# google-deepmind/dqn_zoo

Hardware: NVIDIA H100
Metric: learner_grad_steps_per_sec (higher is better)
Workload: dtype f32 (f64 sum tree)

## Files before the change

### dqn_zoo_b200/_lib.py

```python

import ctypes as C
import os

from dqn_zoo_b200 import _build

i32, i64, f32, f64, u64 = C.c_int32, C.c_int64, C.c_float, C.c_double, C.c_uint64
vp = C.c_void_p

DZ_FLAG_BAD_VALUE, DZ_FLAG_BAD_INDEX, DZ_FLAG_BAD_TARGET, DZ_FLAG_ROOT_ZERO, DZ_FLAG_NONFINITE_WEIGHT = 1, 2, 4, 8, 16
DZ_FLAG_FRAME_POOL_FULL = 32
AGENT_KINDS = {'dqn': 0, 'double_q': 1, 'prioritized': 2, 'c51': 3, 'qrdqn': 4, 'rainbow': 5, 'iqn': 6}
OPTIMIZERS = {'adam': 0, 'rmsprop': 1}


class ReplayView(C.Structure):
  _fields_ = [('d_obs', vp), ('d_action', vp), ('d_reward', vp), ('d_discount', vp), ('capacity', i64),
              ('obs_bytes', i64), ('obs_stride', i64), ('d_tree', vp), ('first_leaf', i64), ('d_live', vp),
              ('d_id_at', vp), ('d_ids', vp), ('d_flags', vp),
              ('d_frames', vp), ('frame_bytes', i64), ('frame_stride', i64), ('obs_channels', i64),
              ('frame_capacity', i64), ('d_planes', vp), ('d_refcount', vp), ('d_hashes', vp), ('d_table', vp),
              ('table_size', i64), ('d_free', vp), ('d_pool_counters', vp), ('d_add_staging', vp)]


class AddRecord(C.Structure):
# ... 86 lines not shown
    'dz_learner_sync_target': (i32, [vp, vp]),
    'dz_test_u8_to_unit': (i32, [vp, vp]),
    'dz_atari_preprocess': (i32, [vp, vp, i32, vp, vp, vp, vp, i32, vp, i32, vp]),
    'dz_atari_preprocess_band_rows': (i32, []),
    'dz_jax_uniform': (i32, [vp, vp, i32, vp, vp]),
    'dz_test_threefry2x32': (i32, [C.c_uint32, C.c_uint32, C.c_uint32, C.c_uint32, vp]),
    'dz_test_learner_buffer': (i32, [vp, C.c_char_p, vp, vp]),
    'dz_test_copy': (i32, [vp, vp, i64, vp]),
    'dz_test_learner_trace': (i32, [vp, C.c_char_p, vp]),
    'dz_test_learner_mma_path': (i32, [vp, C.c_char_p, C.POINTER(i32)]),
    'dz_debug_timeline': (i32, [vp]),
    'dz_test_tc_pgemm_work': (i64, [i32, i32, i32]),
    'dz_test_tc_pgemm': (i32, [vp, i32, i32, i32, vp, i32, i32, i32, i32, i32, vp, vp, i64, i64, i32, i64, vp, i32, vp]),
    'dz_test_umma_gemm': (i32, [vp, i32, vp, i32, i32, i32, i32, i32, vp, i32, i32, vp, i32, vp, vp, vp, vp]),
    'dz_test_umma_gemm_path': (i32, [vp, i32, vp, i32, i32, i32, i32, i32, vp, i32, i32, vp, i32, vp, vp, vp, i32, vp]),
}

EXPORTS = tuple(_SIGNATURES)


def library_path():
  return _build.LIB_PATH


def _load():
  path = library_path()
  if not os.path.exists(path):
    raise ImportError('dqn_zoo_b200: %s is missing — run `python -c "import __graft_entry__ as g; g.build()"` '
                      '(there is no CPU fallback)' % path)
  lib = C.CDLL(path)
# ... 17 lines not shown
```

### dqn_zoo_b200/csrc/dz_tc.cuh

```cuda
#pragma once
#include <cuda_runtime.h>
#include <stdint.h>

namespace dz {
namespace tc {

__device__ __forceinline__ void mma_16x8x8(float (&d)[4], const uint32_t (&a)[4], const uint32_t (&b)[2]) {
  asm volatile("mma.sync.aligned.m16n8k8.row.col.f32.tf32.tf32.f32 {%0, %1, %2, %3}, {%4, %5, %6, %7}, {%8, %9}, {%0, %1, %2, %3};"
               : "+f"(d[0]), "+f"(d[1]), "+f"(d[2]), "+f"(d[3])
               : "r"(a[0]), "r"(a[1]), "r"(a[2]), "r"(a[3]), "r"(b[0]), "r"(b[1]));
}

template <int MT, int NT, class AOff, class BOff>
__device__ __forceinline__ void warp_kstep_3xtf32(float (&sum)[MT][NT][4], const uint8_t* a_hi, const uint8_t* a_lo,
                                                  const uint8_t* b_hi, const uint8_t* b_lo, int m0, int n0, int k0,
                                                  AOff a_off, BOff b_off) {
  const int lane = threadIdx.x & 31, g = lane >> 2, t = lane & 3;
  uint32_t ah[MT][4], al[MT][4];
#pragma unroll
  for (int mt = 0; mt < MT; ++mt) {
#pragma unroll
    for (int q = 0; q < 4; ++q) {
      const uint32_t o = a_off(m0 + mt * 16 + g + (q & 1) * 8, k0 + t + (q >> 1) * 4);
      ah[mt][q] = *reinterpret_cast<const uint32_t*>(a_hi + o);
      al[mt][q] = a_lo ? *reinterpret_cast<const uint32_t*>(a_lo + o) : 0u;
    }
  }
#pragma unroll
  for (int nt = 0; nt < NT; ++nt) {
    uint32_t bh[2], bl[2];
#pragma unroll
    for (int q = 0; q < 2; ++q) {
      const uint32_t o = b_off(n0 + nt * 8 + g, k0 + t + q * 4);
      bh[q] = *reinterpret_cast<const uint32_t*>(b_hi + o);
      bl[q] = *reinterpret_cast<const uint32_t*>(b_lo + o);
    }
#pragma unroll
    for (int mt = 0; mt < MT; ++mt) {
      float p[4] = {0.f, 0.f, 0.f, 0.f};
      if (a_lo) mma_16x8x8(p, al[mt], bh);
      mma_16x8x8(p, ah[mt], bl);
      mma_16x8x8(p, ah[mt], bh);
#pragma unroll
      for (int e = 0; e < 4; ++e) sum[mt][nt][e] += p[e];
    }
  }
}

__device__ __forceinline__ uint64_t wgmma_desc_sw128(uint32_t smem_addr) {
  return (uint64_t)((smem_addr & 0x3FFFFu) >> 4) | ((uint64_t)1 << 16) | ((uint64_t)(1024 >> 4) << 32) | ((uint64_t)1 << 62);
}
__device__ __forceinline__ void wgmma_fence() { asm volatile("wgmma.fence.sync.aligned;" ::: "memory"); }
__device__ __forceinline__ void wgmma_commit() { asm volatile("wgmma.commit_group.sync.aligned;" ::: "memory"); }
template <int N>
__device__ __forceinline__ void wgmma_wait() { asm volatile("wgmma.wait_group.sync.aligned %0;" ::"n"(N) : "memory"); }
template <int NA>
__device__ __forceinline__ void wgmma_fence_acc(float (&d)[NA]) {
#pragma unroll
  for (int e = 0; e < NA; ++e) asm volatile("" : "+f"(d[e])::"memory");
}

// ... 82 lines not shown
```

### dqn_zoo_b200/csrc/dz_umma.cu

```cuda
#include <cudaTypedefs.h>

#include "dz_umma_host.cuh"

namespace dz {

namespace {

PFN_cuTensorMapEncodeTiled_v12000 encode_fn() {
  static PFN_cuTensorMapEncodeTiled_v12000 fn = nullptr;
  if (!fn) {
    void* p = nullptr;
    cudaDriverEntryPointQueryResult q;
    if (cudaGetDriverEntryPoint("cuTensorMapEncodeTiled", &p, cudaEnableDefault, &q) == cudaSuccess && q == cudaDriverEntryPointSuccess)
      fn = reinterpret_cast<PFN_cuTensorMapEncodeTiled_v12000>(p);
  }
  return fn;
}

}

int UmPlan::add_map(const void* base, int rank, const uint64_t* dims, const uint64_t* strides_bytes, const uint32_t* box) {
  auto fn = encode_fn();
  if (!fn) { fail(DZ_ECUDA, "cuTensorMapEncodeTiled entry point not available"); return -1; }
  cuuint64_t gd[5] = {1, 1, 1, 1, 1};
// ... 64 lines not shown
  DZ_CUDA_OK(cudaMalloc(&d_probs, probs.size() * sizeof(UmProblem)));
  DZ_CUDA_OK(cudaMalloc(&d_ctas, ctas.size() * sizeof(UmCta)));
  DZ_CUDA_OK(cudaMalloc(&d_ops, ops.size() * sizeof(UmTmaOp)));
  DZ_CUDA_OK(cudaMemcpy(d_maps, maps.data(), maps.size() * sizeof(CUtensorMap), cudaMemcpyHostToDevice));
  DZ_CUDA_OK(cudaMemcpy(d_probs, probs.data(), probs.size() * sizeof(UmProblem), cudaMemcpyHostToDevice));
  DZ_CUDA_OK(cudaMemcpy(d_ctas, ctas.data(), ctas.size() * sizeof(UmCta), cudaMemcpyHostToDevice));
  DZ_CUDA_OK(cudaMemcpy(d_ops, ops.data(), ops.size() * sizeof(UmTmaOp), cudaMemcpyHostToDevice));
  return DZ_OK;
}

int UmPlan::configure() {
  static bool done = false;
  if (done) return DZ_OK;
  DZ_CUDA_OK(cudaFuncSetAttribute(um::umma_gemm_kernel<32>, cudaFuncAttributeMaxDynamicSharedMemorySize, 227 * 1024));
  DZ_CUDA_OK(cudaFuncSetAttribute(um::umma_gemm_kernel<64>, cudaFuncAttributeMaxDynamicSharedMemorySize, 227 * 1024));
  DZ_CUDA_OK(cudaFuncSetAttribute(um::wgmma_gemm_kernel<32>, cudaFuncAttributeMaxDynamicSharedMemorySize, 227 * 1024));
  DZ_CUDA_OK(cudaFuncSetAttribute(um::wgmma_gemm_kernel<64>, cudaFuncAttributeMaxDynamicSharedMemorySize, 227 * 1024));
  done = true;
  return DZ_OK;
}

bool UmPlan::wgmma_eligible(const UmLaunch& l) const {
  for (int ci = l.cta0; ci < l.cta0 + l.nctas; ++ci) {
    const UmProblem& pr = probs[ctas[ci].prob];
    for (const UmOperand* o : {&pr.A, &pr.B})
      if (o->mn_major || o->nparts != 2 || o->convert) return false;
    if (pr.ksteps != 4) return false;
  }
  return true;
}

int UmPlan::launch(const char* tag, const UmLaunch& l, void* stream, long long* d_trace, int path) const {
  if (l.nctas <= 0) return DZ_OK;
  if (!d_ctas) return fail(DZ_EINVAL, "umma plan not uploaded");
  if (l.stages < 1 || l.stages > um::kStagesMax || l.stage_bytes % 1024) return fail(DZ_EINVAL, "umma launch geometry");
  for (int ci = l.cta0; ci < l.cta0 + l.nctas; ++ci) {
    const UmProblem& pr = probs[ctas[ci].prob];
    const uint32_t want = pr.B.mn_major ? (uint32_t)(l.njt / 32) * pr.B.lbo : (uint32_t)l.njt * 128u;
    if (pr.A.nparts != 2 || pr.B.nparts != 2 || pr.B.part_bytes != want)
      return fail(DZ_EINVAL, "umma launch: operands must be hi/lo pairs and the B tile must span NJT rows");
  }
  for (int ci = l.cta0; ci < l.cta0 + l.nctas; ++ci)
    if (ctas[ci].ops_per_stage > 32) return fail(DZ_EINVAL, "umma launch: more than 32 TMA ops per stage");
  const int stages = l.stages;
  const size_t smem = 1024 + um::kCtlBytes + (size_t)stages * l.stage_bytes;
  if (smem > 227 * 1024) return fail(DZ_EINVAL, "umma launch needs too much shared memory");
  if ((size_t)stages * l.stage_bytes < (size_t)128 * l.njt * 4) return fail(DZ_EINVAL, "umma launch: stage buffers smaller than the store-phase staging tile");
  const int v = l.njt == 32 ? 0 : 1;
  if (l.njt != 32 && l.njt != 64) return fail(DZ_EINVAL, "umma launch: NJT must be 32 or 64");
  if (path != UM_PATH_AUTO && path != UM_PATH_MMA_SYNC && path != UM_PATH_WGMMA) return fail(DZ_EINVAL, "umma launch: unknown MMA path");
  const bool wg = path == UM_PATH_AUTO ? wgmma_eligible(l) : path == UM_PATH_WGMMA;
  if (wg && !wgmma_eligible(l)) return fail(DZ_EINVAL, "umma launch: the wgmma path needs K-major, pre-split operands and four k-steps per stage");
  if (wg)
    for (int ci = l.cta0; ci < l.cta0 + l.nctas; ++ci)
      if (probs[ctas[ci].prob].A.part_bytes + 16384u > l.stage_bytes) return fail(DZ_EINVAL, "umma launch: stage too small for the wgmma A reads");
  DZ_TRY(configure());
  um::UmMaps lm;
  for (int q = 0; q < l.nmaps; ++q) lm.m[q] = maps[l.map_ids[q]];
  for (int q = l.nmaps; q < um::kMaxMapsPerLaunch; ++q) lm.m[q] = maps[l.map_ids[0]];
  if (wg) {
    if (v == 0)
      DZ_LAUNCH_NAMED(tag, um::wgmma_gemm_kernel<32>, (unsigned)l.nctas, um::kThreadsW, smem, stream, lm, d_ctas + l.cta0, d_probs, d_ops, l.nmaps,
                      stages, l.stage_bytes, d_trace);
    else
      DZ_LAUNCH_NAMED(tag, um::wgmma_gemm_kernel<64>, (unsigned)l.nctas, um::kThreadsW, smem, stream, lm, d_ctas + l.cta0, d_probs, d_ops, l.nmaps,
                      stages, l.stage_bytes, d_trace);
    return DZ_OK;
  }
  if (v == 0)
    DZ_LAUNCH_NAMED(tag, um::umma_gemm_kernel<32>, (unsigned)l.nctas, um::kThreadsU, smem, stream, lm, d_ctas + l.cta0, d_probs, d_ops, l.nmaps, stages,
                    l.stage_bytes, d_trace);
  else
    DZ_LAUNCH_NAMED(tag, um::umma_gemm_kernel<64>, (unsigned)l.nctas, um::kThreadsU, smem, stream, lm, d_ctas + l.cta0, d_probs, d_ops, l.nmaps, stages,
                    l.stage_bytes, d_trace);
  return DZ_OK;
}

namespace {
__global__ void um_split_kernel(const float* __restrict__ x, float* __restrict__ hi, float* __restrict__ lo, long long n) {
  dz::pdl_enter();
  long long i = blockIdx.x * (long long)blockDim.x + threadIdx.x;
  if (i < n) {
    float h, l;
// ... 117 lines not shown
```

### dqn_zoo_b200/csrc/dz_umma.cuh

```cuda
#pragma once
#include <cuda.h>

#include "dz_async.cuh"
#include "dz_internal.cuh"
#include "dz_tc.cuh"

namespace dz {

struct UmTmaOp {
  uint32_t map;
  uint32_t smem_off;
  int32_t c[5];
  uint32_t pad;
};

struct UmOperand {
  uint32_t part_bytes;
  uint32_t nparts;
  uint32_t convert;
  uint32_t mn_major;
  uint32_t lbo;
  const float* scale_r;
  const float* scale_i;
};
// ... 17 lines not shown
  int32_t pw;
  int32_t rs_outer, rs_inner;
};

struct UmCta {
  uint32_t prob;
  uint32_t op0;
  uint32_t nstages;
  uint32_t ops_per_stage;
  uint32_t tx_bytes;
  int32_t r0;
  int32_t i0;
  int32_t split;
  int32_t row_base;
  int32_t ph_valid, pw_valid;
  uint32_t pad;
};

namespace um {

using namespace tc;

constexpr int kStagesMax = 8;
constexpr int kConvWarps = 8;
constexpr int kThreadsU = (2 + 4 + kConvWarps) * 32;

__device__ __forceinline__ void convert_part(const UmOperand& o, uint8_t* part0, int r0, int i0, int ct) {
  const int nchunks = (int)(o.part_bytes >> 4);
  const float* __restrict__ sc = o.scale_r;
  const float* __restrict__ si = o.scale_i;
  const int rows_per_slab = (int)(o.lbo >> 7);
// ... 305 lines not shown
        for (int nt = 0; nt < NT; ++nt)
#pragma unroll
          for (int e = 0; e < 4; e += 2) {
            const int r = m0 + frag_row(mt, e), c = frag_col(nt, e);
            *reinterpret_cast<float2*>(reinterpret_cast<float*>(stage_chunk<NJT>(stage_base, r, c >> 2)) + (c & 3)) =
                make_float2(sum[mt][nt][e], sum[mt][nt][e + 1]);
          }
    }
    bar_sync_coop();
    store_tile<NJT>(p, cta, stage_base, threadIdx.x - 64);
  }
  if (tr && warp == 2 && lane == 0) trace[321] = clock64();
  if (tr && threadIdx.x == 0) trace[322] = clock64();
}

constexpr int kThreadsW = 3 * 128;
constexpr int kConsumerWarps = 8;

__device__ __forceinline__ void stamp_if(long long* addr, bool pred) {
  asm volatile("{\n.reg .pred p;\n.reg .b64 c;\nsetp.ne.b32 p, %1, 0;\nmov.u64 c, %%clock64;\n@p st.global.b64 [%0], c;\n}\n" ::"l"(addr),
               "r"((int)pred)
               : "memory");
}

__device__ __forceinline__ int tile_rows_out(const UmProblem& p, const UmCta& c) {
  if (p.epi == UM_EPI_ROWS) {
    if (c.ph_valid <= 0 || c.pw_valid <= 0) return 0;
    const long long n = (long long)(c.ph_valid - 1) * p.pw + min(c.pw_valid, p.pw);
    return (int)min(n, 128LL);
  }
  return max(0, min(128, p.MI - c.i0));
}

template <int NJT>
__global__ void __launch_bounds__(kThreadsW, 1)
    wgmma_gemm_kernel(const __grid_constant__ UmMaps maps, const UmCta* __restrict__ ctas, const UmProblem* __restrict__ probs,
                      const UmTmaOp* __restrict__ ops, int nmaps, int stages, uint32_t stage_bytes, long long* __restrict__ trace) {
  if (threadIdx.x < nmaps) prefetch_tensormap(&maps.m[threadIdx.x]);
// ... 151 lines not shown
```

### dqn_zoo_b200/csrc/dz_umma_host.cuh

```cuda
#pragma once
#include <vector>

#include "dz_umma.cuh"

namespace dz {

enum : int { UM_PATH_AUTO = 0, UM_PATH_MMA_SYNC = 1, UM_PATH_WGMMA = 2 };

struct UmLaunch {
  int cta0 = 0, nctas = 0;
  int njt = 64;
  int stages = 4;
  uint32_t stage_bytes = 0;
  int nmaps = 0;
  int map_ids[um::kMaxMapsPerLaunch] = {0};
};

struct UmPlan {
  std::vector<CUtensorMap> maps;
  std::vector<UmProblem> probs;
  std::vector<UmCta> ctas;
  std::vector<UmTmaOp> ops;
  CUtensorMap* d_maps = nullptr;
  UmProblem* d_probs = nullptr;
  UmCta* d_ctas = nullptr;
  UmTmaOp* d_ops = nullptr;

  int add_map(const void* base, int rank, const uint64_t* dims, const uint64_t* strides_bytes, const uint32_t* box);
  int localize_maps(UmLaunch& l);
  int upload();
  void release();
  int launch(const char* tag, const UmLaunch& l, void* stream, long long* d_trace = nullptr, int path = UM_PATH_AUTO) const;
  bool wgmma_eligible(const UmLaunch& l) const;
  int path_of(const UmLaunch& l) const { return wgmma_eligible(l) ? UM_PATH_WGMMA : UM_PATH_MMA_SYNC; }
  static int configure();
};

inline UmOperand um_kmajor(int rows, bool hi_lo, bool convert, const float* scale_r = nullptr) {
  UmOperand o;
  memset(&o, 0, sizeof(o));
  o.part_bytes = (uint32_t)(((rows * 128) + 1023) / 1024 * 1024);
  o.nparts = hi_lo ? 2 : 1; o.convert = convert ? 1 : 0; o.mn_major = 0; o.lbo = 0; o.scale_r = scale_r;
  return o;
}
inline UmOperand um_mnmajor(int mn, int r_rows, bool convert, const float* scale_r = nullptr) {
  UmOperand o;
  memset(&o, 0, sizeof(o));
  o.lbo = (uint32_t)(r_rows * 128);
// ... 7 lines not shown
```

### dqn_zoo_b200/csrc/dz_umma_net.cu

```cuda
#include <algorithm>

#include "dz_umma_net.cuh"

namespace dz {

struct UmNet {
  UmNetDesc d;
  int h1, w1, h2, w2, h3, w3, feat, PB;
  int njt_fc;
  UmPlan plan;
  float *act_hi[3], *act_lo[3], *act_f32[3];
  float *dact_hi[3], *dact_lo[3], *dact_f32[3];
  float *h1_buf, *dh1_f32, *dh1_hi, *dh1_lo;
  float *fc_part, *fcd_part;
  int fc_splits, fcd_splits, fc_nprob, fcd_nsrc;
  float *wf_hi[2][3], *wf_lo[2][3], *wd3_hi, *wd3_lo, *wd2_hi, *wd2_lo;
  int map_wf1[2][2];
  UmLaunch l_conv2, l_conv3, l_dconv3, l_dconv2, l_fc, l_fcd, l_wconv3, l_wconv2;
  float *wg3_part, *wg2_part, *wg1_part;
  int wg3_splits, wg2_splits, wg1_ctas;
  int map_g1[2];
  float* wg_scratch;
  unsigned int* wg_ticket;
  int conv1_stag_bytes, conv1_tiles_per_pass;
  struct Patch { int prob; int field; int64_t off; };
  std::vector<Patch> patches;
  const float* noise_cached = nullptr;
  std::string trace_tag;
  long long* trace_ptr = nullptr;
  long long* tr(const char* tag) const { return trace_ptr && trace_tag == tag ? trace_ptr : nullptr; }
};

namespace {

using namespace um;

struct PackArgs {
  const float* blob[2];
  int64_t off_w[3];
  float* wf_hi[2][3]; float* wf_lo[2][3];
  float *wd3_hi, *wd3_lo, *wd2_hi, *wd2_lo;
};

__global__ void __launch_bounds__(256) um_pack_conv_kernel(const __grid_constant__ PackArgs a) {
  dz::pdl_enter();
// ... 924 lines not shown

  n->l_fc.nctas = 0; n->l_fcd.nctas = 0;
  if (d.use_fc) {
    const int njt = B <= 32 ? 32 : 64;
    n->njt_fc = njt;
    const int q = d.noisy ? 2 : 1;
    int m_x[2], m_g[2];
    for (int part = 0; part < 2; ++part) {
      uint64_t dims[2] = {(uint64_t)feat, (uint64_t)PB}, strides[1] = {(uint64_t)feat * 4};
      uint32_t box[2] = {32, (uint32_t)njt};
      m_x[part] = pl.add_map(part ? n->act_lo[2] : n->act_hi[2], 2, dims, strides, box);
      uint64_t gd[2] = {512, (uint64_t)d.nstream * B}, gs[1] = {2048};
      m_g[part] = pl.add_map(part ? n->dh1_lo : n->dh1_hi, 2, gd, gs, box);
      if (m_x[part] < 0 || m_g[part] < 0) return DZ_EINVAL;
    }
    int m_wf_fc[2][2][2], m_wd_fc[2][2];
    bool wf3d = true;
    for (int blob = 0; blob < 2; ++blob)
      for (int s = 0; s < d.nstream; ++s)
        for (int sg = 0; sg < q; ++sg) {
          const float* w = (blob ? d.target : d.online) + (sg ? d.off_fc_sw[s] : d.off_fc_w[s]);
          uint64_t dims[2] = {512, (uint64_t)feat}, strides[1] = {2048};
          uint64_t dims3[3] = {32, (uint64_t)feat, 16}, strides3[2] = {2048, 128};
          uint32_t box3[3] = {32, 32, 4};
          if (wf3d) {
            m_wf_fc[blob][s][sg] = pl.add_map(w, 3, dims3, strides3, box3);
            if (m_wf_fc[blob][s][sg] < 0) wf3d = false;
          }
          if (!wf3d) {
            if (blob || s || sg) return fail(DZ_EINVAL, "fc weight tensor maps: inconsistent encodings");
            uint32_t box2[2] = {32, 32};
            m_wf_fc[blob][s][sg] = pl.add_map(w, 2, dims, strides, box2);
          }
          if (m_wf_fc[blob][s][sg] < 0) return DZ_EINVAL;
          if (blob == 0) {
            uint32_t boxd[2] = {32, 128};
            m_wd_fc[s][sg] = pl.add_map(w, 2, dims, strides, boxd);
            if (m_wd_fc[s][sg] < 0) return DZ_EINVAL;
          }
        }
    {
      UmOperand Bo = um_kmajor(njt, true, false);
      const int nk = feat / 32, S = n->fc_splits, per = (nk + S - 1) / S;
      n->l_fc.cta0 = (int)pl.ctas.size(); n->l_fc.njt = njt;
      n->l_fc.stage_bytes = 2 * 16384 + 2 * Bo.part_bytes;
      n->l_fc.stages = std::min<int>(kStagesMax, (int)((226 * 1024 - 1024 - kCtlBytes) / n->l_fc.stage_bytes));
      for (int p = 0; p < d.npass; ++p) {
        const int blob = d.pass_target[p] ? 1 : 0;
        for (int s = 0; s < d.nstream; ++s) {
          const int qi = p * d.nstream + s;
          UmProblem pr;
          memset(&pr, 0, sizeof(pr));
          pr.A = um_mnmajor(128, 32, true, nullptr); pr.B = Bo; pr.ksteps = 4; pr.red_per_stage = 32;
          if (d.noisy) pr.A.convert = 2;
          pr.epi = UM_EPI_PARTIAL; pr.MI = 512; pr.NJ = B;
          pr.C = n->fc_part + (int64_t)qi * S * B * 512; pr.sc_i = 1; pr.sc_j = 512; pr.split_stride = (long long)B * 512;
          const int prob = (int)pl.probs.size();
          pl.probs.push_back(pr);
          if (d.noisy) {
            n->patches.push_back({prob, 0, (int64_t)d.noise_apply[p] * d.noise_stride + d.noise_off_in[s]});
            n->patches.push_back({prob, 2, (int64_t)d.noise_apply[p] * d.noise_stride + d.noise_off_out[s]});
          }
          for (int sp = 0; sp < S; ++sp)
            for (int nt = 0; nt < 4; ++nt) {
              const int k0 = sp * per, k1 = std::min(nk, k0 + per);
              if (k1 <= k0) continue;
              UmCta c;
              memset(&c, 0, sizeof(c));
              c.prob = (uint32_t)prob; c.op0 = (uint32_t)pl.ops.size(); c.nstages = (uint32_t)(k1 - k0);
              c.ops_per_stage = (wf3d ? 1 : 4) * (d.noisy ? 2 : 1) + 2;
              c.tx_bytes = (uint32_t)((d.noisy ? 32768 : 16384) + 2 * njt * 128);
              c.r0 = 32 * k0; c.i0 = nt * 128; c.split = sp;
              for (int ks = k0; ks < k1; ++ks) {
                for (int sg = 0; sg < (d.noisy ? 2 : 1); ++sg) {
                  if (wf3d) push_op(pl, m_wf_fc[blob][s][sg], sg * 16384, 0, 32 * ks, nt * 4, 0, 0);
                  else for (int sl = 0; sl < 4; ++sl) push_op(pl, m_wf_fc[blob][s][sg], sg * 16384 + sl * 4096, nt * 128 + 32 * sl, 32 * ks, 0, 0, 0);
                }
                for (int part = 0; part < 2; ++part) push_op(pl, m_x[part], 32768 + part * Bo.part_bytes, 32 * ks, p * B, 0, 0, 0);
              }
              pl.ctas.push_back(c);
            }
        }
      }
      n->l_fc.nctas = (int)pl.ctas.size() - n->l_fc.cta0;
    }
    {
      UmOperand Bo = um_kmajor(njt, true, false);
      const int S = n->fcd_splits, per = (16 + S - 1) / S, ktiles = (feat + 127) / 128;
      n->l_fcd.cta0 = (int)pl.ctas.size(); n->l_fcd.njt = njt;
      n->l_fcd.stage_bytes = 2 * 16384 + 2 * Bo.part_bytes;
      n->l_fcd.stages = std::min<int>(kStagesMax, (int)((226 * 1024 - 1024 - kCtlBytes) / n->l_fcd.stage_bytes));
      for (int s = 0; s < d.nstream; ++s) {
        UmProblem pr;
// ... 43 lines not shown
  }
  DZ_CUDA_OK(cudaStreamSynchronize((cudaStream_t)stream));
  DZ_CUDA_OK(cudaMemcpy(n->plan.d_probs, n->plan.probs.data(), n->plan.probs.size() * sizeof(UmProblem), cudaMemcpyHostToDevice));
  n->noise_cached = noise;
  return DZ_OK;
}

}

int64_t um_net_workspace_bytes(const UmNetDesc& d) {
  UmNet tmp;
  tmp.d = d;
  return carve_net(&tmp, nullptr);
}

int um_net_create(const UmNetDesc& d, char* base, UmNet** out) {
  if (!um_net_supported(d)) return fail(DZ_EINVAL, "geometry not supported by the tensor-core path");
  UmNet* n = new UmNet();
  n->d = d;
  carve_net(n, base);
  const int px = n->h1 * n->w1, m_pass = d.B * px;
  n->conv1_tiles_per_pass = (m_pass + 127) / 128;
  int worst = 0;
  for (int m0 = 0; m0 < m_pass; m0 += 128) {
    const int m1 = std::min(m0 + 128, m_pass);
    int tot = 0;
    for (int b = m0 / px; b <= (m1 - 1) / px; ++b) tot += conv1_segment(b, m0, m1, px, n->w1, d.W * 4).bytes;
    worst = std::max(worst, tot);
  }
  n->conv1_stag_bytes = (worst + 127) / 128 * 128;
  cudaMemset(n->wg_ticket, 0, 64 * 4);
  for (int L = 0; L < 3; ++L) {
    const int64_t cnt[3] = {(int64_t)d.B * n->h1 * n->w1 * 32, (int64_t)d.B * n->h2 * n->w2 * 64, (int64_t)d.B * n->feat};
    cudaMemset(n->dact_hi[L], 0, cnt[L] * 4); cudaMemset(n->dact_lo[L], 0, cnt[L] * 4); cudaMemset(n->dact_f32[L], 0, cnt[L] * 4);
// ... 5 lines not shown
  if (rc == DZ_OK) rc = n->plan.upload();
  if (rc == DZ_OK) rc = UmPlan::configure();
  if (rc != DZ_OK) { um_net_destroy(n); return rc; }
  static bool configured = false;
  if (!configured) {
    if (cudaFuncSetAttribute(conv1_umma_kernel, cudaFuncAttributeMaxDynamicSharedMemorySize, 227 * 1024) != cudaSuccess ||
        cudaFuncSetAttribute(conv1_wgrad_umma_kernel, cudaFuncAttributeMaxDynamicSharedMemorySize, 227 * 1024) != cudaSuccess) {
      um_net_destroy(n);
      return fail(DZ_ECUDA, "conv1_umma_kernel shared memory attribute");
    }
    configured = true;
  }
  *out = n;
  return DZ_OK;
}

void um_net_trace(UmNet* n, const char* tag, long long* d_trace) { n->trace_tag = tag ? tag : ""; n->trace_ptr = d_trace; }

int um_net_mma_path(UmNet* n, const char* tag) {
  const std::string t = tag ? tag : "";
  const UmLaunch* l = t == "conv2_fwd" ? &n->l_conv2 : t == "conv3_fwd" ? &n->l_conv3 : t == "conv3_dgrad" ? &n->l_dconv3
                    : t == "conv2_dgrad" ? &n->l_dconv2 : (t == "fc1_fwd" || t == "noisy1_fwd") ? &n->l_fc
                    : (t == "fc1_dgrad" || t == "noisy1_dgrad") ? &n->l_fcd : t == "conv3_wgrad" ? &n->l_wconv3
                    : t == "conv2_wgrad" ? &n->l_wconv2 : nullptr;
  if (!l || l->nctas <= 0) return -1;
  return n->plan.path_of(*l);
}

void um_net_destroy(UmNet* n) {
  if (!n) return;
// ... 121 lines not shown
  else if (layer == 2) f = WgFinish{n->wg2_part, n->wg2_splits, 512 * 64, 512 * 64, dW, n->dact_f32[1], n->d.B * n->h2 * n->w2, 64, db, sc + 256 * 64, n->wg_ticket + 1, 0, nullptr};
  else f = WgFinish{n->wg1_part, n->wg1_ctas, 256 * 32, 256 * 32, dW, n->dact_f32[0], n->d.B * n->h1 * n->w1, 32, db, sc + 2 * 256 * 64, n->wg_ticket + 2, 0, nullptr};
  f.sum_blocks = wg_sum_blocks(layer);
  f.norm_part = norm_parts ? norm_parts + wg_slot_base(layer) : nullptr;
  const int chunks = (f.M + kWgChunkRows - 1) / kWgChunkRows;
  if (chunks > kWgMaxChunks) return fail(DZ_EINVAL, "bias-gradient reduction: too many row chunks");
  const char* tags[3] = {"wgrad_finish1", "wgrad_finish2", "wgrad_finish3"};
  DZ_LAUNCH_NAMED(tags[layer - 1], um_wgrad_finish_kernel, (unsigned)(f.sum_blocks + chunks), 256, 0, stream, f);
  return DZ_OK;
}

int um_backward_conv3(UmNet* n, void* stream) { return n->plan.launch("conv3_dgrad", n->l_dconv3, stream, n->tr("conv3_dgrad")); }
int um_backward_conv2(UmNet* n, void* stream) { return n->plan.launch("conv2_dgrad", n->l_dconv2, stream, n->tr("conv2_dgrad")); }

}
```

### include/dqn_zoo_b200.h

```cpp
#ifndef DQN_ZOO_B200_H_
#define DQN_ZOO_B200_H_

#include <stddef.h>
#include <stdint.h>

#ifdef __cplusplus
extern "C" {
#endif

#define DZ_OK 0
#define DZ_EINVAL (-1)
#define DZ_ECUDA (-2)
#define DZ_ERANGE (-3)
#define DZ_ESTATE (-4)

const char* dz_last_error(void);
const char* dz_build_info(void);
int64_t dz_launch_count(void);
int dz_profile_begin(void);
int dz_profile_end(char* out, int64_t cap);


int dz_sumtree_rebuild(double* d_nodes, int64_t first_leaf, int64_t n_valid, void* stream);

// ... 208 lines not shown
int dz_test_copy(void* d_dst, const void* d_src, int64_t bytes, void* stream);
int dz_test_learner_trace(dz_learner* l, const char* tag, long long* d_trace);
int dz_test_learner_mma_path(dz_learner* l, const char* tag, int32_t* path);
int dz_debug_timeline(unsigned long long* d_buf);
int64_t dz_test_tc_pgemm_work(int32_t a_rows, int32_t b_rows, int32_t red);
int dz_test_tc_pgemm(const float* d_A, int32_t a_rows, int32_t a_ld, int32_t a_red_contig, const float* d_B,
                     int32_t b_rows, int32_t b_ld, int32_t b_red_contig, int32_t red, int32_t a_ones_row,
                     float* d_work, float* d_C, int64_t sc_i, int64_t sc_j, int32_t splits, int64_t split_stride,
                     const float* d_bias, int32_t relu, void* stream);
int dz_test_umma_gemm(const float* d_A, int32_t a_mn_major, const float* d_B, int32_t b_mn_major, int32_t MI, int32_t NJ,
                      int32_t R, int32_t convert, const float* d_scale_r, int32_t stages, int32_t epi_rows,
                      const float* d_bias, int32_t relu, float* d_C, float* d_hi, float* d_lo, void* stream);
int dz_test_umma_gemm_path(const float* d_A, int32_t a_mn_major, const float* d_B, int32_t b_mn_major, int32_t MI, int32_t NJ,
                           int32_t R, int32_t convert, const float* d_scale_r, int32_t stages, int32_t epi_rows,
                           const float* d_bias, int32_t relu, float* d_C, float* d_hi, float* d_lo, int32_t path, void* stream);

#ifdef __cplusplus
}
#endif
#endif
```

Measured before the change: 2684.

## Share FC weight tiles across passes using one blob in a dedicated fc kernel

Forward passes that apply the same parameter blob (online or target) are grouped so that one CTA serves up to two problems. Each weight tile is then loaded once by TMA and multiplied against both passes' activations. A new warp-specialized umma_fc_kernel has one producer warp and eight mma.sync warps; it applies the noisy-net weight transform in registers and runs a 3xTF32 split product, which is factored into a reusable warp helper. The aim is to cut redundant FC1 weight traffic. The cost is a smaller row tile per CTA, with more CTAs but less data per CTA, and additional eligibility logic.

```diff
diff --git a/dqn_zoo_b200/_lib.py b/dqn_zoo_b200/_lib.py
--- a/dqn_zoo_b200/_lib.py
+++ b/dqn_zoo_b200/_lib.py
@@ -124,6 +124,8 @@
     'dz_test_tc_pgemm': (i32, [vp, i32, i32, i32, vp, i32, i32, i32, i32, i32, vp, vp, i64, i64, i32, i64, vp, i32, vp]),
     'dz_test_umma_gemm': (i32, [vp, i32, vp, i32, i32, i32, i32, i32, vp, i32, i32, vp, i32, vp, vp, vp, vp]),
     'dz_test_umma_gemm_path': (i32, [vp, i32, vp, i32, i32, i32, i32, i32, vp, i32, i32, vp, i32, vp, vp, vp, i32, vp]),
+    'dz_test_fc_forward': (i32, [i32, i32, i32, i32, i32, i32, vp, vp, vp, vp, vp, i64, vp, vp, vp, i32, vp, C.POINTER(i32),
+                                 C.POINTER(i64), vp]),
 }
 
 EXPORTS = tuple(_SIGNATURES)
diff --git a/dqn_zoo_b200/csrc/dz_tc.cuh b/dqn_zoo_b200/csrc/dz_tc.cuh
--- a/dqn_zoo_b200/csrc/dz_tc.cuh
+++ b/dqn_zoo_b200/csrc/dz_tc.cuh
@@ -9,6 +9,31 @@
   asm volatile("mma.sync.aligned.m16n8k8.row.col.f32.tf32.tf32.f32 {%0, %1, %2, %3}, {%4, %5, %6, %7}, {%8, %9}, {%0, %1, %2, %3};"
                : "+f"(d[0]), "+f"(d[1]), "+f"(d[2]), "+f"(d[3])
                : "r"(a[0]), "r"(a[1]), "r"(a[2]), "r"(a[3]), "r"(b[0]), "r"(b[1]));
+}
+
+template <int MT, int NT, class BOff>
+__device__ __forceinline__ void warp_mma_3xtf32(float (&sum)[MT][NT][4], const uint32_t (&ah)[MT][4], const uint32_t (&al)[MT][4],
+                                                bool a_has_lo, const uint8_t* b_hi, const uint8_t* b_lo, int n0, int k0, BOff b_off) {
+  const int lane = threadIdx.x & 31, g = lane >> 2, t = lane & 3;
+#pragma unroll
+  for (int nt = 0; nt < NT; ++nt) {
+    uint32_t bh[2], bl[2];
+#pragma unroll
+    for (int q = 0; q < 2; ++q) {
+      const uint32_t o = b_off(n0 + nt * 8 + g, k0 + t + q * 4);
+      bh[q] = *reinterpret_cast<const uint32_t*>(b_hi + o);
+      bl[q] = *reinterpret_cast<const uint32_t*>(b_lo + o);
+    }
+#pragma unroll
+    for (int mt = 0; mt < MT; ++mt) {
+      float p[4] = {0.f, 0.f, 0.f, 0.f};
+      if (a_has_lo) mma_16x8x8(p, al[mt], bh);
+      mma_16x8x8(p, ah[mt], bl);
+      mma_16x8x8(p, ah[mt], bh);
+#pragma unroll
+      for (int e = 0; e < 4; ++e) sum[mt][nt][e] += p[e];
+    }
+  }
 }
 
 template <int MT, int NT, class AOff, class BOff>
@@ -26,25 +51,7 @@
       al[mt][q] = a_lo ? *reinterpret_cast<const uint32_t*>(a_lo + o) : 0u;
     }
   }
-#pragma unroll
-  for (int nt = 0; nt < NT; ++nt) {
-    uint32_t bh[2], bl[2];
-#pragma unroll
-    for (int q = 0; q < 2; ++q) {
-      const uint32_t o = b_off(n0 + nt * 8 + g, k0 + t + q * 4);
-      bh[q] = *reinterpret_cast<const uint32_t*>(b_hi + o);
-      bl[q] = *reinterpret_cast<const uint32_t*>(b_lo + o);
-    }
-#pragma unroll
-    for (int mt = 0; mt < MT; ++mt) {
-      float p[4] = {0.f, 0.f, 0.f, 0.f};
-      if (a_lo) mma_16x8x8(p, al[mt], bh);
-      mma_16x8x8(p, ah[mt], bl);
-      mma_16x8x8(p, ah[mt], bh);
-#pragma unroll
-      for (int e = 0; e < 4; ++e) sum[mt][nt][e] += p[e];
-    }
-  }
+  warp_mma_3xtf32<MT, NT>(sum, ah, al, a_lo != nullptr, b_hi, b_lo, n0, k0, b_off);
 }
 
 __device__ __forceinline__ uint64_t wgmma_desc_sw128(uint32_t smem_addr) {
diff --git a/dqn_zoo_b200/csrc/dz_umma.cu b/dqn_zoo_b200/csrc/dz_umma.cu
--- a/dqn_zoo_b200/csrc/dz_umma.cu
+++ b/dqn_zoo_b200/csrc/dz_umma.cu
@@ -102,6 +102,8 @@
   if (done) return DZ_OK;
   DZ_CUDA_OK(cudaFuncSetAttribute(um::umma_gemm_kernel<32>, cudaFuncAttributeMaxDynamicSharedMemorySize, 227 * 1024));
   DZ_CUDA_OK(cudaFuncSetAttribute(um::umma_gemm_kernel<64>, cudaFuncAttributeMaxDynamicSharedMemorySize, 227 * 1024));
+  DZ_CUDA_OK(cudaFuncSetAttribute(um::umma_fc_kernel<32>, cudaFuncAttributeMaxDynamicSharedMemorySize, 227 * 1024));
+  DZ_CUDA_OK(cudaFuncSetAttribute(um::umma_fc_kernel<64>, cudaFuncAttributeMaxDynamicSharedMemorySize, 227 * 1024));
   DZ_CUDA_OK(cudaFuncSetAttribute(um::wgmma_gemm_kernel<32>, cudaFuncAttributeMaxDynamicSharedMemorySize, 227 * 1024));
   DZ_CUDA_OK(cudaFuncSetAttribute(um::wgmma_gemm_kernel<64>, cudaFuncAttributeMaxDynamicSharedMemorySize, 227 * 1024));
   done = true;
@@ -114,6 +116,26 @@
     for (const UmOperand* o : {&pr.A, &pr.B})
       if (o->mn_major || o->nparts != 2 || o->convert) return false;
     if (pr.ksteps != 4) return false;
+  }
+  return true;
+}
+
+bool UmPlan::fc_eligible(const UmLaunch& l) const {
+  for (int ci = l.cta0; ci < l.cta0 + l.nctas; ++ci) {
+    const UmCta& c = ctas[ci];
+    const int np = c.nprob > 1 ? (int)c.nprob : 1;
+    if (np > um::kFcMaxProbs) return false;
+    for (int q = 0; q < np; ++q) {
+      const UmProblem& pr = probs[c.prob + q];
+      if (!pr.A.mn_major || pr.A.lbo != 4096u || pr.A.part_bytes * (uint32_t)np != 16384u) return false;
+      if (pr.A.convert != 2 && !(pr.A.convert == 1 && pr.A.scale_r == nullptr)) return false;
+      if (pr.B.mn_major || pr.B.nparts != 2 || pr.B.convert) return false;
+      if (pr.ksteps != 4 || pr.red_per_stage != 32 || pr.epi != UM_EPI_PARTIAL || pr.sc_i != 1) return false;
+      if (q > 0 && (pr.A.part_bytes != probs[c.prob].A.part_bytes || pr.A.convert != probs[c.prob].A.convert ||
+                    pr.B.part_bytes != probs[c.prob].B.part_bytes))
+        return false;
+    }
+    if (2 * 16384u / (uint32_t)np + (uint32_t)np * 2u * probs[c.prob].B.part_bytes > l.stage_bytes) return false;
   }
   return true;
 }
@@ -136,7 +158,8 @@
   if ((size_t)stages * l.stage_bytes < (size_t)128 * l.njt * 4) return fail(DZ_EINVAL, "umma launch: stage buffers smaller than the store-phase staging tile");
   const int v = l.njt == 32 ? 0 : 1;
   if (l.njt != 32 && l.njt != 64) return fail(DZ_EINVAL, "umma launch: NJT must be 32 or 64");
-  if (path != UM_PATH_AUTO && path != UM_PATH_MMA_SYNC && path != UM_PATH_WGMMA) return fail(DZ_EINVAL, "umma launch: unknown MMA path");
+  if (path != UM_PATH_AUTO && path != UM_PATH_MMA_SYNC && path != UM_PATH_WGMMA && path != UM_PATH_CONVERTERS)
+    return fail(DZ_EINVAL, "umma launch: unknown MMA path");
   const bool wg = path == UM_PATH_AUTO ? wgmma_eligible(l) : path == UM_PATH_WGMMA;
   if (wg && !wgmma_eligible(l)) return fail(DZ_EINVAL, "umma launch: the wgmma path needs K-major, pre-split operands and four k-steps per stage");
   if (wg)
@@ -155,6 +178,17 @@
                       stages, l.stage_bytes, d_trace);
     return DZ_OK;
   }
+  if (path != UM_PATH_CONVERTERS && fc_eligible(l)) {
+    if (v == 0)
+      DZ_LAUNCH_NAMED(tag, um::umma_fc_kernel<32>, (unsigned)l.nctas, um::kThreadsF, smem, stream, lm, d_ctas + l.cta0, d_probs, d_ops, l.nmaps,
+                      stages, l.stage_bytes, d_trace);
+    else
+      DZ_LAUNCH_NAMED(tag, um::umma_fc_kernel<64>, (unsigned)l.nctas, um::kThreadsF, smem, stream, lm, d_ctas + l.cta0, d_probs, d_ops, l.nmaps,
+                      stages, l.stage_bytes, d_trace);
+    return DZ_OK;
+  }
+  for (int ci = l.cta0; ci < l.cta0 + l.nctas; ++ci)
+    if (ctas[ci].nprob > 1) return fail(DZ_EINVAL, "umma launch: CTAs that serve several problems need umma_fc_kernel");
   if (v == 0)
     DZ_LAUNCH_NAMED(tag, um::umma_gemm_kernel<32>, (unsigned)l.nctas, um::kThreadsU, smem, stream, lm, d_ctas + l.cta0, d_probs, d_ops, l.nmaps, stages,
                     l.stage_bytes, d_trace);
diff --git a/dqn_zoo_b200/csrc/dz_umma.cuh b/dqn_zoo_b200/csrc/dz_umma.cuh
--- a/dqn_zoo_b200/csrc/dz_umma.cuh
+++ b/dqn_zoo_b200/csrc/dz_umma.cuh
@@ -55,7 +55,7 @@
   int32_t split;
   int32_t row_base;
   int32_t ph_valid, pw_valid;
-  uint32_t pad;
+  uint32_t nprob;
 };
 
 namespace um {
@@ -391,14 +391,157 @@
   if (tr && threadIdx.x == 0) trace[322] = clock64();
 }
 
-constexpr int kThreadsW = 3 * 128;
-constexpr int kConsumerWarps = 8;
-
 __device__ __forceinline__ void stamp_if(long long* addr, bool pred) {
   asm volatile("{\n.reg .pred p;\n.reg .b64 c;\nsetp.ne.b32 p, %1, 0;\nmov.u64 c, %%clock64;\n@p st.global.b64 [%0], c;\n}\n" ::"l"(addr),
                "r"((int)pred)
                : "memory");
 }
+
+constexpr int kFcMmaWarps = 8;
+constexpr int kThreadsF = (1 + kFcMmaWarps) * 32;
+constexpr int kFcMaxProbs = 2;
+
+template <int NJT>
+__global__ void __launch_bounds__(kThreadsF, 1)
+    umma_fc_kernel(const __grid_constant__ UmMaps maps, const UmCta* __restrict__ ctas, const UmProblem* __restrict__ probs,
+                   const UmTmaOp* __restrict__ ops, int nmaps, int stages, uint32_t stage_bytes, long long* __restrict__ trace) {
+  if (threadIdx.x < nmaps) prefetch_tensormap(&maps.m[threadIdx.x]);
+  extern __shared__ uint8_t smem_raw[];
+  uint8_t* smem = smem_raw + smem_pad_1024(smem_raw);
+  const bool tr = trace != nullptr && blockIdx.x == 0;
+  const UmCta cta = ctas[blockIdx.x];
+  const int ST = stages;
+  const int nst = (int)cta.nstages;
+  const int P = cta.nprob > 1 ? 2 : 1;
+
+  uint64_t* full = reinterpret_cast<uint64_t*>(smem);
+  uint64_t* empty = full + 2 * kStagesMax;
+  UmProblem* p_smem = reinterpret_cast<UmProblem*>(smem + 1024);
+  UmTmaOp* ops_smem = reinterpret_cast<UmTmaOp*>(smem + 2048);
+  uint8_t* stage_base = smem + kCtlBytes;
+  static_assert(kFcMaxProbs * sizeof(UmProblem) <= 1024, "problem copies do not fit their slot");
+
+  const int warp = threadIdx.x >> 5, lane = threadIdx.x & 31;
+  {
+    const uint4* src = reinterpret_cast<const uint4*>(probs + cta.prob);
+    uint4* dst = reinterpret_cast<uint4*>(p_smem);
+    for (int i = threadIdx.x; i < P * (int)(sizeof(UmProblem) / 16); i += kThreadsF) dst[i] = src[i];
+    const int nvec = min(nst * (int)cta.ops_per_stage, kMaxOpsPerCta) * 2;
+    const uint4* osrc = reinterpret_cast<const uint4*>(ops + cta.op0);
+    uint4* odst = reinterpret_cast<uint4*>(ops_smem);
+    for (int i = threadIdx.x; i < nvec; i += kThreadsF) odst[i] = osrc[i];
+  }
+  if (warp == 0 && lane == 0) {
+    for (int s = 0; s < ST; ++s) { mbar_init(&full[s], 1); mbar_init(&empty[s], kFcMmaWarps); }
+    fence_mbarrier_init();
+  }
+  __syncthreads();
+
+  if (warp == 0) {
+    const int nops = (int)cta.ops_per_stage;
+    int s = 0;
+    uint32_t ph = 0;
+    uint32_t st_addr = smem_u32(stage_base);
+    int oi = 0;
+    dz::pdl_enter();
+    if (tr && lane == 0) { trace[323] = clock64(); trace[324] = clock64(); }
+    for (int it = 0; it < nst; ++it) {
+      mbar_wait(&empty[s], ph ^ 1u);
+      if (lane == 0) mbar_expect_tx(&full[s], cta.tx_bytes);
+      __syncwarp();
+      if (lane < nops) {
+        const int o = oi + lane;
+        const UmTmaOp op = o < kMaxOpsPerCta ? ops_smem[o] : ops[cta.op0 + o];
+        tma_load_5d(st_addr + op.smem_off, &maps.m[op.map], &full[s], op.c[0], op.c[1], op.c[2], op.c[3], op.c[4]);
+      }
+      if (tr && lane == 0 && it < 64) trace[it] = clock64();
+      __syncwarp();
+      oi += nops;
+      ++s; st_addr += stage_bytes;
+      if (s == ST) { s = 0; ph ^= 1u; st_addr = smem_u32(stage_base); }
+    }
+    return;
+  }
+
+  const int w = warp - 1, wpp = kFcMmaWarps / P;
+  const int q = w / wpp, m0 = 16 * (w - q * wpp);
+  const bool lead = w == 0 && lane == 0;
+  const UmProblem& p = p_smem[q];
+  const int g = lane >> 2, t = lane & 3;
+  const uint32_t a_part = p.A.part_bytes, a_lbo = p.A.lbo;
+  const uint8_t* b_first = stage_base + a_part * 2 + (uint32_t)q * 2u * p.B.part_bytes;
+  const uint32_t b_part = p.B.part_bytes;
+  const bool noisy = p.A.convert == 2;
+  const float* __restrict__ eps_in = p.A.scale_r;
+  constexpr int NT = NJT / 8;
+  float sum[1][NT][4];
+#pragma unroll
+  for (int nt = 0; nt < NT; ++nt)
+#pragma unroll
+    for (int e = 0; e < 4; ++e) sum[0][nt][e] = 0.f;
+  auto b_off = [](int n, int k) { return sw128_kmajor(n, k); };
+  dz::pdl_enter();
+  float eo[2] = {1.f, 1.f};
+  if (noisy) {
+    eo[0] = p.A.scale_i[cta.i0 + m0 + g];
+    eo[1] = p.A.scale_i[cta.i0 + m0 + g + 8];
+  }
+  int s = 0, r0 = cta.r0;
+  uint32_t ph = 0;
+  for (int it = 0; it < nst; ++it) {
+    mbar_wait(&full[s], ph);
+    stamp_if(trace + 64 + it, tr && lead && it < 64);
+    const uint8_t* mu = stage_base + (size_t)s * stage_bytes;
+    const uint8_t* sg = mu + a_part;
+    const uint8_t* bh = b_first + (size_t)s * stage_bytes;
+#pragma unroll(NJT == 32 ? 4 : 2)
+    for (int ks = 0; ks < 4; ++ks) {
+      uint32_t ah[1][4], al[1][4];
+      float ei[2] = {1.f, 1.f};
+      if (noisy) { ei[0] = eps_in[r0 + 8 * ks + t]; ei[1] = eps_in[r0 + 8 * ks + t + 4]; }
+#pragma unroll
+      for (int e = 0; e < 4; ++e) {
+        const uint32_t o = sw128_mnmajor(m0 + g + (e & 1) * 8, 8 * ks + t + (e >> 1) * 4, a_lbo);
+        float v = *reinterpret_cast<const float*>(mu + o);
+        if (noisy) {
+          const float f = ei[e >> 1] * eo[e & 1];
+          v = fmaf(*reinterpret_cast<const float*>(sg + o), f, v);
+        }
+        float hh, ll;
+        split_tf32(v, hh, ll);
+        ah[0][e] = __float_as_uint(hh);
+        al[0][e] = __float_as_uint(ll);
+      }
+      warp_mma_3xtf32<1, NT>(sum, ah, al, true, bh, bh + b_part, 0, 8 * ks, b_off);
+    }
+    __syncwarp();
+    if (lane == 0) mbar_arrive(&empty[s]);
+    stamp_if(trace + 128 + it, tr && lead && it < 64);
+    r0 += 32;
+    if (++s == ST) { s = 0; ph ^= 1u; }
+  }
+  if (lead) asm volatile("griddepcontrol.launch_dependents;" ::: "memory");
+  if (tr && lead) trace[320] = clock64();
+  float* dst = p.C + (long long)cta.split * p.split_stride;
+  const long long sc_j = p.sc_j;
+#pragma unroll
+  for (int e = 0; e < 4; e += 2) {
+    const int i = cta.i0 + m0 + frag_row(0, e);
+    if (i >= p.MI) continue;
+    const float sc = p.scale_i ? p.scale_i[i] : 1.0f;
+#pragma unroll
+    for (int nt = 0; nt < NT; ++nt)
+#pragma unroll
+      for (int h = 0; h < 2; ++h) {
+        const int j = frag_col(nt, e + h);
+        if (j < p.NJ) dst[i + (long long)j * sc_j] = sum[0][nt][e + h] * sc;
+      }
+  }
+  if (tr && lead) { trace[321] = clock64(); trace[322] = clock64(); }
+}
+
+constexpr int kThreadsW = 3 * 128;
+constexpr int kConsumerWarps = 8;
 
 __device__ __forceinline__ int tile_rows_out(const UmProblem& p, const UmCta& c) {
   if (p.epi == UM_EPI_ROWS) {
diff --git a/dqn_zoo_b200/csrc/dz_umma_host.cuh b/dqn_zoo_b200/csrc/dz_umma_host.cuh
--- a/dqn_zoo_b200/csrc/dz_umma_host.cuh
+++ b/dqn_zoo_b200/csrc/dz_umma_host.cuh
@@ -5,7 +5,7 @@
 
 namespace dz {
 
-enum : int { UM_PATH_AUTO = 0, UM_PATH_MMA_SYNC = 1, UM_PATH_WGMMA = 2 };
+enum : int { UM_PATH_AUTO = 0, UM_PATH_MMA_SYNC = 1, UM_PATH_WGMMA = 2, UM_PATH_CONVERTERS = 3 };
 
 struct UmLaunch {
   int cta0 = 0, nctas = 0;
@@ -32,6 +32,7 @@
   void release();
   int launch(const char* tag, const UmLaunch& l, void* stream, long long* d_trace = nullptr, int path = UM_PATH_AUTO) const;
   bool wgmma_eligible(const UmLaunch& l) const;
+  bool fc_eligible(const UmLaunch& l) const;
   int path_of(const UmLaunch& l) const { return wgmma_eligible(l) ? UM_PATH_WGMMA : UM_PATH_MMA_SYNC; }
   static int configure();
 };
diff --git a/dqn_zoo_b200/csrc/dz_umma_net.cu b/dqn_zoo_b200/csrc/dz_umma_net.cu
--- a/dqn_zoo_b200/csrc/dz_umma_net.cu
+++ b/dqn_zoo_b200/csrc/dz_umma_net.cu
@@ -29,6 +29,7 @@
   std::string trace_tag;
   long long* trace_ptr = nullptr;
   long long* tr(const char* tag) const { return trace_ptr && trace_tag == tag ? trace_ptr : nullptr; }
+  bool fc_per_pass = false;
 };
 
 namespace {
@@ -983,6 +984,18 @@
       m_g[part] = pl.add_map(part ? n->dh1_lo : n->dh1_hi, 2, gd, gs, box);
       if (m_x[part] < 0 || m_g[part] < 0) return DZ_EINVAL;
     }
+    int grp[3][kFcMaxProbs], ngrp = 0, grp_n[3] = {0, 0, 0}, grp_blob[3] = {0, 0, 0};
+    for (int p = 0; p < d.npass; ++p) {
+      const int blob = d.pass_target[p] ? 1 : 0;
+      int gi = -1;
+      if (!n->fc_per_pass)
+        for (int k = 0; k < ngrp; ++k) if (grp_blob[k] == blob) gi = k;
+      if (gi < 0) { gi = ngrp++; grp_blob[gi] = blob; }
+      if (grp_n[gi] == kFcMaxProbs) return fail(DZ_EINVAL, "fc forward: more than two passes apply one parameter blob");
+      grp[gi][grp_n[gi]++] = p;
+    }
+    int fc_rows[2] = {128, 128};
+    for (int k = 0; k < ngrp; ++k) fc_rows[grp_blob[k]] = 128 / grp_n[k];
     int m_wf_fc[2][2][2], m_wd_fc[2][2];
     bool wf3d = true;
     for (int blob = 0; blob < 2; ++blob)
@@ -991,7 +1004,7 @@
           const float* w = (blob ? d.target : d.online) + (sg ? d.off_fc_sw[s] : d.off_fc_w[s]);
           uint64_t dims[2] = {512, (uint64_t)feat}, strides[1] = {2048};
           uint64_t dims3[3] = {32, (uint64_t)feat, 16}, strides3[2] = {2048, 128};
-          uint32_t box3[3] = {32, 32, 4};
+          uint32_t box3[3] = {32, 32, (uint32_t)fc_rows[blob] / 32};
           if (wf3d) {
             m_wf_fc[blob][s][sg] = pl.add_map(w, 3, dims3, strides3, box3);
             if (m_wf_fc[blob][s][sg] < 0) wf3d = false;
@@ -1013,39 +1026,48 @@
       const int nk = feat / 32, S = n->fc_splits, per = (nk + S - 1) / S;
       n->l_fc.cta0 = (int)pl.ctas.size(); n->l_fc.njt = njt;
       n->l_fc.stage_bytes = 2 * 16384 + 2 * Bo.part_bytes;
+      for (int k = 0; k < ngrp; ++k)
+        n->l_fc.stage_bytes = std::max<uint32_t>(n->l_fc.stage_bytes, 2 * 16384 / grp_n[k] + grp_n[k] * 2 * Bo.part_bytes);
       n->l_fc.stages = std::min<int>(kStagesMax, (int)((226 * 1024 - 1024 - kCtlBytes) / n->l_fc.stage_bytes));
-      for (int p = 0; p < d.npass; ++p) {
-        const int blob = d.pass_target[p] ? 1 : 0;
+      for (int k = 0; k < ngrp; ++k) {
+        const int blob = grp_blob[k], np = grp_n[k], rows = fc_rows[blob], slabs = rows / 32;
+        const UmOperand A = um_mnmajor(rows, 32, true, nullptr);
+        const uint32_t a_bytes = 2 * A.part_bytes;
         for (int s = 0; s < d.nstream; ++s) {
-          const int qi = p * d.nstream + s;
-          UmProblem pr;
-          memset(&pr, 0, sizeof(pr));
-          pr.A = um_mnmajor(128, 32, true, nullptr); pr.B = Bo; pr.ksteps = 4; pr.red_per_stage = 32;
-          if (d.noisy) pr.A.convert = 2;
-          pr.epi = UM_EPI_PARTIAL; pr.MI = 512; pr.NJ = B;
-          pr.C = n->fc_part + (int64_t)qi * S * B * 512; pr.sc_i = 1; pr.sc_j = 512; pr.split_stride = (long long)B * 512;
-          const int prob = (int)pl.probs.size();
-          pl.probs.push_back(pr);
-          if (d.noisy) {
-            n->patches.push_back({prob, 0, (int64_t)d.noise_apply[p] * d.noise_stride + d.noise_off_in[s]});
-            n->patches.push_back({prob, 2, (int64_t)d.noise_apply[p] * d.noise_stride + d.noise_off_out[s]});
+          const int prob0 = (int)pl.probs.size();
+          for (int gp = 0; gp < np; ++gp) {
+            const int p = grp[k][gp], qi = p * d.nstream + s;
+            UmProblem pr;
+            memset(&pr, 0, sizeof(pr));
+            pr.A = A; pr.B = Bo; pr.ksteps = 4; pr.red_per_stage = 32;
+            if (d.noisy) pr.A.convert = 2;
+            pr.epi = UM_EPI_PARTIAL; pr.MI = 512; pr.NJ = B;
+            pr.C = n->fc_part + (int64_t)qi * S * B * 512; pr.sc_i = 1; pr.sc_j = 512; pr.split_stride = (long long)B * 512;
+            const int prob = (int)pl.probs.size();
+            pl.probs.push_back(pr);
+            if (d.noisy) {
+              n->patches.push_back({prob, 0, (int64_t)d.noise_apply[p] * d.noise_stride + d.noise_off_in[s]});
+              n->patches.push_back({prob, 2, (int64_t)d.noise_apply[p] * d.noise_stride + d.noise_off_out[s]});
+            }
           }
           for (int sp = 0; sp < S; ++sp)
-            for (int nt = 0; nt < 4; ++nt) {
+            for (int nt = 0; nt < 512 / rows; ++nt) {
               const int k0 = sp * per, k1 = std::min(nk, k0 + per);
               if (k1 <= k0) continue;
               UmCta c;
               memset(&c, 0, sizeof(c));
-              c.prob = (uint32_t)prob; c.op0 = (uint32_t)pl.ops.size(); c.nstages = (uint32_t)(k1 - k0);
-              c.ops_per_stage = (wf3d ? 1 : 4) * (d.noisy ? 2 : 1) + 2;
-              c.tx_bytes = (uint32_t)((d.noisy ? 32768 : 16384) + 2 * njt * 128);
-              c.r0 = 32 * k0; c.i0 = nt * 128; c.split = sp;
+              c.prob = (uint32_t)prob0; c.nprob = (uint32_t)np; c.op0 = (uint32_t)pl.ops.size(); c.nstages = (uint32_t)(k1 - k0);
+              c.ops_per_stage = (wf3d ? 1 : slabs) * q + 2 * np;
+              c.tx_bytes = (uint32_t)(q * A.part_bytes + np * 2 * njt * 128);
+              c.r0 = 32 * k0; c.i0 = nt * rows; c.split = sp;
               for (int ks = k0; ks < k1; ++ks) {
-                for (int sg = 0; sg < (d.noisy ? 2 : 1); ++sg) {
-                  if (wf3d) push_op(pl, m_wf_fc[blob][s][sg], sg * 16384, 0, 32 * ks, nt * 4, 0, 0);
-                  else for (int sl = 0; sl < 4; ++sl) push_op(pl, m_wf_fc[blob][s][sg], sg * 16384 + sl * 4096, nt * 128 + 32 * sl, 32 * ks, 0, 0, 0);
+                for (int sg = 0; sg < q; ++sg) {
+                  if (wf3d) push_op(pl, m_wf_fc[blob][s][sg], sg * A.part_bytes, 0, 32 * ks, nt * slabs, 0, 0);
+                  else for (int sl = 0; sl < slabs; ++sl) push_op(pl, m_wf_fc[blob][s][sg], sg * A.part_bytes + sl * 4096, nt * rows + 32 * sl, 32 * ks, 0, 0, 0);
                 }
-                for (int part = 0; part < 2; ++part) push_op(pl, m_x[part], 32768 + part * Bo.part_bytes, 32 * ks, p * B, 0, 0, 0);
+                for (int gp = 0; gp < np; ++gp)
+                  for (int part = 0; part < 2; ++part)
+                    push_op(pl, m_x[part], a_bytes + (gp * 2 + part) * Bo.part_bytes, 32 * ks, grp[k][gp] * B, 0, 0, 0);
               }
               pl.ctas.push_back(c);
             }
@@ -1119,10 +1141,12 @@
   return carve_net(&tmp, nullptr);
 }
 
-int um_net_create(const UmNetDesc& d, char* base, UmNet** out) {
+namespace {
+int net_create(const UmNetDesc& d, char* base, UmNet** out, bool fc_per_pass) {
   if (!um_net_supported(d)) return fail(DZ_EINVAL, "geometry not supported by the tensor-core path");
   UmNet* n = new UmNet();
   n->d = d;
+  n->fc_per_pass = fc_per_pass;
   carve_net(n, base);
   const int px = n->h1 * n->w1, m_pass = d.B * px;
   n->conv1_tiles_per_pass = (m_pass + 127) / 128;
@@ -1158,6 +1182,9 @@
   *out = n;
   return DZ_OK;
 }
+}
+
+int um_net_create(const UmNetDesc& d, char* base, UmNet** out) { return net_create(d, base, out, false); }
 
 void um_net_trace(UmNet* n, const char* tag, long long* d_trace) { n->trace_tag = tag ? tag : ""; n->trace_ptr = d_trace; }
 
@@ -1309,3 +1336,50 @@
 int um_backward_conv2(UmNet* n, void* stream) { return n->plan.launch("conv2_dgrad", n->l_dconv2, stream, n->tr("conv2_dgrad")); }
 
 }
+
+using namespace dz;
+
+extern "C" int dz_test_fc_forward(int32_t B, int32_t H, int32_t W, int32_t npass, int32_t nstream, int32_t noisy, const float* online,
+                                  const float* target, const int64_t* off_w, const int64_t* off_sw, const float* noise,
+                                  int64_t noise_stride, const int64_t* off_in, const int64_t* off_out, const float* x, int32_t per_pass,
+                                  float* d_part, int32_t* splits, int64_t* weight_bytes, void* stream) {
+  if (nstream < 1 || nstream > 2 || npass < 1 || npass > 3) return fail(DZ_EINVAL, "fc forward test: npass 1..3, nstream 1..2");
+  UmNetDesc d;
+  memset(&d, 0, sizeof(d));
+  d.B = B; d.H = H; d.W = W; d.npass = npass;
+  d.pass_target[0] = 0; d.pass_target[1] = npass == 3 ? 0 : 1; d.pass_target[2] = 1;
+  d.online = online; d.target = target;
+  d.use_fc = 1; d.nstream = nstream; d.noisy = noisy ? 1 : 0;
+  for (int s = 0; s < nstream; ++s) {
+    d.off_fc_w[s] = off_w[s];
+    if (noisy) { d.off_fc_sw[s] = off_sw[s]; d.noise_off_in[s] = off_in[s]; d.noise_off_out[s] = off_out[s]; }
+  }
+  for (int p = 0; p < 3; ++p) d.noise_apply[p] = p;
+  d.noise_stride = noise_stride;
+  if (!um_net_supported(d)) return fail(DZ_EINVAL, "fc forward test: geometry not supported by the tensor-core path");
+  char* ws = nullptr;
+  DZ_CUDA_OK(cudaMalloc(&ws, (size_t)um_net_workspace_bytes(d)));
+  UmNet* n = nullptr;
+  int rc = net_create(d, ws, &n, per_pass != 0);
+  if (rc == DZ_OK) rc = um_split(x, n->act_hi[2], n->act_lo[2], (long long)n->PB * n->feat, stream);
+  if (rc == DZ_OK && noisy) rc = apply_noise(n, noise, stream);
+  if (rc == DZ_OK) rc = n->plan.launch("fc1_fwd", n->l_fc, stream, nullptr, per_pass ? UM_PATH_CONVERTERS : UM_PATH_AUTO);
+  if (rc == DZ_OK) {
+    const size_t bytes = (size_t)npass * nstream * n->fc_splits * B * 512 * sizeof(float);
+    if (cudaMemcpyAsync(d_part, n->fc_part, bytes, cudaMemcpyDeviceToDevice, (cudaStream_t)stream) != cudaSuccess ||
+        cudaStreamSynchronize((cudaStream_t)stream) != cudaSuccess)
+      rc = fail(DZ_ECUDA, "fc forward test: %s", cudaGetErrorString(cudaGetLastError()));
+  }
+  if (rc == DZ_OK) {
+    *splits = n->fc_splits;
+    int64_t wb = 0;
+    for (int ci = n->l_fc.cta0; ci < n->l_fc.cta0 + n->l_fc.nctas; ++ci) {
+      const UmCta& c = n->plan.ctas[ci];
+      wb += (int64_t)c.nstages * (noisy ? 2 : 1) * n->plan.probs[c.prob].A.part_bytes;
+    }
+    *weight_bytes = wb;
+  }
+  if (n) um_net_destroy(n);
+  cudaFree(ws);
+  return rc;
+}
diff --git a/include/dqn_zoo_b200.h b/include/dqn_zoo_b200.h
--- a/include/dqn_zoo_b200.h
+++ b/include/dqn_zoo_b200.h
@@ -246,6 +246,10 @@
 int dz_test_umma_gemm_path(const float* d_A, int32_t a_mn_major, const float* d_B, int32_t b_mn_major, int32_t MI, int32_t NJ,
                            int32_t R, int32_t convert, const float* d_scale_r, int32_t stages, int32_t epi_rows,
                            const float* d_bias, int32_t relu, float* d_C, float* d_hi, float* d_lo, int32_t path, void* stream);
+int dz_test_fc_forward(int32_t B, int32_t H, int32_t W, int32_t npass, int32_t nstream, int32_t noisy, const float* online,
+                       const float* target, const int64_t* off_w, const int64_t* off_sw, const float* noise, int64_t noise_stride,
+                       const int64_t* off_in, const int64_t* off_out, const float* x, int32_t per_pass, float* d_part,
+                       int32_t* splits, int64_t* weight_bytes, void* stream);
 
 #ifdef __cplusplus
 }
```

Measured after the change: 2858, median of 6. 1.06x the previous value.
